# francescobrigante/Audio-Style-Transfer

Hardware: AMD Instinct MI355X
Metric: audio-seconds/sec/node (train step, 4s@22.05kHz pairs) (higher is better)
Workload: dtype bf16; 1 GPU; configs[1]: batch=8 4 s clips per GPU (S=2, x=(B,S,2,287,597)), full train2 step: STFT + CQT front-end from resident waveforms, encoders+decoder+discriminator, all losses, D and G phases, grad clip, Adam; global_batch=8, parallelism=dp1, hip_graph=True, dp_semantics=per-rank BN and batch-coupled losses

## Files before the change

audio-style-transfer_amd/ast_amd/ops.py:

```python
from __future__ import annotations

import ctypes
import functools
import math

import torch

from . import _lib, config
from ._lib import Gather, check, dcode, len_tensor, lib, ptr, stream


@functools.lru_cache(maxsize=None)
def const_tensor(values, dtype, device):
    return torch.tensor(values, dtype=dtype, device=device)


def pad8(c: int) -> int:
    return (c + 7) // 8 * 8


def _tap(dh, dw, wt):
    return (dh + 64) | ((dw + 64) << 8) | (wt << 16)


def _mk(N, Hs, Ws, Cs, Hm, Wm, sh, sw, oh, ow, Hd, Wd, Cd, dsh, dsw, doh, dow, taps, wtaps):
    g = Gather(N=N, Hs=Hs, Ws=Ws, Cs=Cs, Hm=Hm, Wm=Wm, sh=sh, sw=sw, oh=oh, ow=ow, Hd=Hd, Wd=Wd, Cd=Cd,
               dsh=dsh, dsw=dsw, doh=doh, dow=dow, ntaps=len(taps), wtaps=wtaps)
    for i, (dh, dw, wt) in enumerate(taps):
        g.tap[i] = _tap(dh, dw, wt)
    return g


@functools.lru_cache(maxsize=None)
def gather_direct(N, H, W, Cs, Cd, k, stride, pad):
    Ho = (H + 2 * pad - k) // stride + 1
    Wo = (W + 2 * pad - k) // stride + 1
    taps = tuple((kh, kw, kh * k + kw) for kh in range(k) for kw in range(k))
    return _mk(N, H, W, Cs, Ho, Wo, stride, stride, -pad, -pad, Ho, Wo, Cd, 1, 1, 0, 0, taps, k * k), (Ho, Wo)


@functools.lru_cache(maxsize=None)
def gathers_transposed(N, Hs, Ws, Cs, Hd, Wd, Cd, k, stride, pad):
    out = []
    for ph in range(stride):
        th = [((ph + pad - kh) // stride, kh) for kh in range(k) if (ph + pad - kh) % stride == 0]
        Hm = (Hd - ph + stride - 1) // stride
        for pw in range(stride):
            tw = [((pw + pad - kw) // stride, kw) for kw in range(k) if (pw + pad - kw) % stride == 0]
            Wm = (Wd - pw + stride - 1) // stride
            if Hm <= 0 or Wm <= 0:
                continue
            taps = tuple((dh, dw, kh * k + kw) for dh, kh in th for dw, kw in tw)
            out.append(_mk(N, Hs, Ws, Cs, Hm, Wm, 1, 1, 0, 0, Hd, Wd, Cd, stride, stride, ph, pw, taps, k * k))
    return tuple(out)


PROFILE = None


def _gemm_cost(g, esize, wgrad=False):
    M = g.N * g.Hm * g.Wm
    K = g.ntaps * g.Cs
    flops = 2.0 * M * g.Cd * K
    if wgrad:
        nbytes = (M * g.Cd + g.N * g.Hs * g.Ws * g.Cs) * esize + g.Cd * K * 4
    else:
        src_pix = min(g.N * g.Hs * g.Ws, M * max(g.ntaps, 1))
        nbytes = (src_pix * g.Cs + M * g.Cd + g.Cd * K) * esize
    return flops, nbytes


def _igemm_plan(g, dt):
    out = (ctypes.c_int32 * 5)()
    check(lib().ast_igemm_plan(g, dt, ctypes.byref(out)), "ast_igemm_plan")
    return out


def _igemm_config(g, dt):
    out = _igemm_plan(g, dt)
    if out[2] < 0:
        return f"patch{-out[0]}r{'(rows,' + str(-out[3]) + 'frag)' if out[3] < 0 else ''},{out[1]}ch,slab{-out[2]}B"
    return f"{out[0]}x{out[1]},k{out[2] * 16}B" + (f",split{out[3]}" if out[3] > 1 else "") + (f",kg{out[4]}" if out[4] > 1 else "")


_ws_cache = {}


def _ws_need(g, dt):
    det = config.deterministic
    key = (id(g), dt, det)
    v = _ws_cache.get(key)
    if v is None:
        v = int(lib().ast_igemm_ws_floats_det(g, dt) if det else lib().ast_igemm_ws_floats(g, dt))
        check(min(v, 0), "ast_igemm_ws_floats")
        _ws_cache[key] = v
    return v


STAT_SLOTS = 64


def stat_slots(C):
    s = STAT_SLOTS
    while s > 8 and s * C > 4096:
        s //= 2
    return s


def _slot_flags(slots):
    return 0 if slots == 64 else ((slots.bit_length() - 1) << _lib.IGEMM_SLOTS_SHIFT)


class _StatArena:
    CAP = 1 << 24
    by_device = {}


def stat_table(n, device):
    device = torch.device(device)
    a = _StatArena.by_device.get(device)
    if a is None:
        a = _StatArena.by_device[device] = [torch.zeros(_StatArena.CAP, dtype=torch.float32, device=device), 0, 0]
    n64 = (int(n) + 63) // 64 * 64
    if a[1] + n64 > _StatArena.CAP:
        if torch.cuda.is_current_stream_capturing():
            raise RuntimeError("statistics arena exhausted inside a hipGraph capture: call ops.stat_arena_reset() at the start of the step")
        torch.cuda.synchronize(device)
        a[0].zero_()
        a[1] = 0
    t = a[0][a[1]:a[1] + int(n)]
    a[1] += n64
    a[2] = max(a[2], a[1])
    return t


def stat_arena_reset(device):
    a = _StatArena.by_device.get(torch.device(device))
    if a is None or a[2] == 0:
        return
    if config.fused_finalize or _SyncBN.active:
        a[0][:a[2]].zero_()
    a[1] = 0


def stats_fusable(g, dt):
    return _ws_need(g, dt) == 0 and not config.deterministic


class BNLink:
    __slots__ = ("x", "scale", "shift", "relu", "table", "filled", "slots")

    def __init__(self):
        self.x = self.scale = self.shift = self.table = None
        self.relu, self.filled, self.slots = True, False, STAT_SLOTS


def in_stats_fusable(g, dt):
    return _igemm_plan(g, dt)[2] != 0 and _ws_need(g, dt) == 0 and not config.deterministic


def _igemm(src, wgt, bias, dst, g, flags=0, stats=None, bn=None, per_image=False):
    if PROFILE is not None:
        e0, e1 = torch.cuda.Event(enable_timing=True), torch.cuda.Event(enable_timing=True)
        e0.record()
# ... 1355 lines not shown
```

audio-style-transfer_amd/csrc/igemm.hip:

```cpp
#include "gemm_common.h"

namespace {


__device__ __forceinline__ int swz(int row, int c) { return ((c + (((row >> 3) & 1) << 1)) & 3) << 4; }

template <typename T>
struct EpiCtx {
  T* dst; const float* bias; float* ws; const T* bn_x; const float* bn_scale; const float* bn_shift;
  int HWm; float rcp_hw, rcp_w; bool accumulate, relu, stats, bstats, bn_relu;
};

template <typename T, int TN, int MODE>
__device__ __forceinline__ void epi_store_m(const EpiCtx<T>& ec, const ast_gather_t& g, const f32x4 (&col)[TN], const size_t pix, const int co0,
                                            float (&st1)[TN][4], float (&st2)[TN][4]) {
  T* drow = ec.dst + pix * g.Cd;
#pragma unroll
  for (int i = 0; i < TN; ++i) {
    const int co = co0 + i * 16;
    if (co >= g.Cd) continue;
    float v[4];
#pragma unroll
    for (int r = 0; r < 4; ++r) v[r] = col[i][r];
    if (ec.bias) {
// ... 376 lines not shown
  const int nks = (nchunks + 3) >> 2;
  const int HWm = g.Hm * g.Wm;
  const __amdgpu_buffer_rsrc_t srcR = __builtin_amdgcn_make_buffer_rsrc((void*)src, 0, src_bytes, 0x00020000);
  const __amdgpu_buffer_rsrc_t wgtR = __builtin_amdgcn_make_buffer_rsrc((void*)wgt, 0, wgt_bytes, 0x00020000);

  int sdelta[NKS], tdh[NKS], tdw[NKS];
  unsigned woff[NKS];
#pragma unroll
  for (int ks = 0; ks < NKS; ++ks) {
    const int kc = ks * 4 + fq;
    const bool kval = kc < nchunks;
    const int t = kval ? (cpc_shift >= 0 ? (kc >> cpc_shift) : kc / cpc) : 0;
    const int c0b = (kc - t * cpc) * 16;
    int dh, dw, wt;
    decode_tap(taptab[t], dh, dw, wt);
    sdelta[ks] = (dh * g.Ws + dw) * g.Cs * ES + c0b;
    tdh[ks] = kval ? dh : (1 << 20);
    tdw[ks] = dw;
    woff[ks] = kval ? (unsigned)(wt * g.Cs * ES + c0b) : OOB;
  }
  frag wreg[TN][NKS];
#pragma unroll
  for (int i = 0; i < TN; ++i) {
    const int co = bn0 + i * 16 + fr;
    const unsigned rowoff = co < g.Cd ? (unsigned)(co * g.wtaps * g.Cs * ES) : OOB;
#pragma unroll
    for (int ks = 0; ks < NKS; ++ks)
      wreg[i][ks] = __builtin_bit_cast(frag, __builtin_amdgcn_raw_buffer_load_b128(wgtR, (rowoff != OOB && woff[ks] != OOB) ? rowoff + woff[ks] : OOB, 0, 0));
  }

  const bool accumulate = flags & AST_IGEMM_ACCUMULATE, relu = flags & AST_IGEMM_RELU, stats = !DET && (flags & AST_IGEMM_STATS), bstats = !DET && (flags & AST_IGEMM_BN_SUMS), bn_relu = !(flags & AST_IGEMM_BN_NO_RELU);
  EpiCtx<T> ec{dst, bias, ws, bn_x, bn_scale, bn_shift, HWm, rcp_hw, rcp_w, accumulate, relu, stats, bstats, bn_relu};
  float st1[TN][4], st2[TN][4];
#pragma unroll
  for (int i = 0; i < TN; ++i)
#pragma unroll
    for (int r = 0; r < 4; ++r) { st1[i][r] = 0.f; st2[i][r] = 0.f; }

  auto load_pix = [&](int j, u32x4 (&xr)[NKS], int& dpix) __attribute__((always_inline)) {
    const int m = bm0 + j * 16 + fr;
    const bool valid = j < jt && m < M;
    const int mm = valid ? m : 0;
    const int n = fdiv(mm, HWm, rcp_hw), rem = mm - n * HWm;
    const int hm = fdiv(rem, g.Wm, rcp_w), wq = rem - hm * g.Wm;
    const int hs0 = valid ? hm * g.sh + g.oh : -(1 << 20);
    const int ws0 = wq * g.sw + g.ow;
    const int roff = (((n * g.Hs + (valid ? hs0 : 0)) * g.Ws + ws0) * g.Cs) * ES;
    dpix = (n * g.Hd + hm * g.dsh + g.doh) * g.Wd + (wq * g.dsw + g.dow);
#pragma unroll
    for (int ks = 0; ks < NKS; ++ks) {
      const bool ok = (unsigned)(hs0 + tdh[ks]) < (unsigned)g.Hs && (unsigned)(ws0 + tdw[ks]) < (unsigned)g.Ws;
      xr[ks] = __builtin_amdgcn_raw_buffer_load_b128(srcR, ok ? (unsigned)(roff + sdelta[ks]) : OOB, 0, 0);
    }
  };
  auto compute = [&](int j, const u32x4 (&xr)[NKS], const int dpix) __attribute__((always_inline)) {
    f32x4 acc[TN];
#pragma unroll
    for (int i = 0; i < TN; ++i) acc[i] = f32x4{0.f, 0.f, 0.f, 0.f};
#pragma unroll
    for (int ks = 0; ks < NKS; ++ks) {
      if (ks < nks) {
        const frag xf = __builtin_bit_cast(frag, xr[ks]);
#pragma unroll
        for (int i = 0; i < TN; ++i) acc[i] = Mma<T>::run(wreg[i][ks], xf, acc[i]);
      }
    }
    const int m = bm0 + j * 16 + fr;
    if (m < M) epi_store<T, TN>(ec, g, acc, (size_t)dpix, bn0 + fq * 4, st1, st2);
  };

  u32x4 xa[NKS], xb[NKS];
  int pa, pb;
  load_pix(0, xa, pa);
  for (int j = 0; j < jt; j += 2) {
    load_pix(j + 1, xb, pb);
    compute(j, xa, pa);
    load_pix(j + 2, xa, pa);
    if (j + 1 < jt) compute(j + 1, xb, pb);
  }
  __shared__ float red[(TN + 1) / 2 * 256];
  if (stats || bstats) epi_flush<T, TN>(ec, g, st1, st2, tix & stat_slot_mask(flags), bn0, fr, fq, red);
}

template <typename T>
__global__ __launch_bounds__(256) void splitk_finish_kernel(float* __restrict__ ws, const float* __restrict__ bias,
                                                            T* __restrict__ dst, const ast_gather_t g, const int M, const int flags,
                                                            const int nslabs) {
  const int c4 = g.Cd >> 2;
  const int HWm = g.Hm * g.Wm;
  const size_t total = (size_t)M * c4;
  for (size_t i = (size_t)blockIdx.x * 256 + threadIdx.x; i < total; i += (size_t)gridDim.x * 256) {
    const int m = (int)(i / c4), co = (int)(i % c4) * 4;
    const int n = m / HWm, rem = m - n * HWm;
    const int hm = rem / g.Wm, wq = rem - hm * g.Wm;
    const size_t pix = (size_t)(n * g.Hd + hm * g.dsh + g.doh) * g.Wd + (wq * g.dsw + g.dow);
    f32x4* wp = reinterpret_cast<f32x4*>(ws + (size_t)m * g.Cd + co);
    f32x4 a = *wp;
    if (nslabs > 0) {
      for (int z = 1; z < nslabs; ++z) a += *reinterpret_cast<const f32x4*>(ws + ((size_t)z * M + m) * g.Cd + co);
    } else {
      *wp = f32x4{0.f, 0.f, 0.f, 0.f};
    }
    float v[4] = {a[0], a[1], a[2], a[3]};
    if (bias) for (int r = 0; r < 4; ++r) v[r] += bias[co + r];
    store4<T>(dst + pix * g.Cd + co, v, flags & AST_IGEMM_ACCUMULATE, flags & AST_IGEMM_RELU);
  }
}

constexpr int PC_MAXPL = 8;

#ifdef AST_STAMPS
__device__ unsigned long long ast_stamps[16384 * 8];
#define PC_STAMP(k) do { if (threadIdx.x == 0 && tix < 16384) ast_stamps[tix * 8 + (k)] = (k) >= 6 ? wall_clock64() : __builtin_readcyclecounter(); } while (0)
#else
#define PC_STAMP(k) do { } while (0)
#endif
struct PconvPlan { int TH, TWF, PH, PW, dhmin, dwmin, tiles_h, tiles_w, nct, lds, rows, tm, wall; unsigned m_nct, m_per_img, m_tiles_w, m_pw20, m_twf, m_twf20; unsigned long long tapq[3]; };
__host__ __device__ __forceinline__ unsigned pc_magic(int d) { return d <= 1 ? 0u : (unsigned)((0x100000000ull + (unsigned)d - 1) / (unsigned)d); }
__device__ __forceinline__ int pc_div(int n, int d, unsigned m) { return d == 1 ? n : (int)__umulhi((unsigned)n, m); }
__device__ __forceinline__ int pc_div20(int n, unsigned m20) { return (int)(__umul24((unsigned)n, m20) >> 20); }

template <int SLB> __device__ __forceinline__ int pc_h(int p) { return SLB == 128 ? (p & 7) : ((p >> 1) & 3); }

typedef __attribute__((ext_vector_type(2))) unsigned int u32x2;
__device__ __forceinline__ f32x4 pc_as_f32x4(u32x4 u) {
  return __builtin_bit_cast(f32x4, u);
}
template <typename T>
__device__ __forceinline__ f32x4 pc_load4(__amdgpu_buffer_rsrc_t r, unsigned voff, int imm) {
  if constexpr (sizeof(T) == 4) {
    return pc_as_f32x4(__builtin_amdgcn_raw_buffer_load_b128(r, voff + (unsigned)imm, 0, 0));
  } else {
    const u32x2 u = __builtin_amdgcn_raw_buffer_load_b64(r, voff + (unsigned)imm, 0, 0);
    const u32x4 w{u.x << 16, u.x & 0xffff0000u, u.y << 16, u.y & 0xffff0000u};
    return __builtin_bit_cast(f32x4, w);
  }
}
template <typename T>
__device__ __forceinline__ void pc_store4(__amdgpu_buffer_rsrc_t r, unsigned voff, int imm, f32x4 v) {
  if constexpr (sizeof(T) == 4) {
    __builtin_amdgcn_raw_buffer_store_b128(__builtin_bit_cast(u32x4, v), r, voff + (unsigned)imm, 0, 0);
  } else {
    const bf16x4 q{(bf16_t)v[0], (bf16_t)v[1], (bf16_t)v[2], (bf16_t)v[3]};
    __builtin_amdgcn_raw_buffer_store_b64(__builtin_bit_cast(u32x2, q), r, voff + (unsigned)imm, 0, 0);
  }
}

template <typename T, int SLB, int TM, int TN, bool WALL, bool DET>
__global__ __launch_bounds__(256, (WALL ? 2 : (TM * TN <= 8 ? 4 : 2))) void pconv_kernel(const T* __restrict__ src, const T* __restrict__ wgt, const float* __restrict__ bias,
                                                    T* __restrict__ dst, const ast_gather_t g, const PconvPlan pp, const int flags,
                                                    float* __restrict__ ws, const unsigned src_bytes, const unsigned wgt_bytes,
                                                    const T* __restrict__ bn_x, const float* __restrict__ bn_scale,
                                                    const float* __restrict__ bn_shift) {
  constexpr int ES = sizeof(T);
  constexpr int CPP = SLB / 16;
  constexpr int BN = TN * 16;
  constexpr int NWL = (BN * CPP + 255) / 256;
  constexpr int KS = SLB / 64;
  constexpr unsigned OOB = 0x80000000u;
  using frag = typename Mma<T>::frag;
  extern __shared__ __attribute__((aligned(16))) unsigned char pl[];
  const int patch_bytes = pp.PH * pp.PW * SLB;
  unsigned char* wbuf = pl + patch_bytes;

  const int tid = threadIdx.x, lane = tid & 63, wave = tid >> 6;
  const int fr = lane & 15, fq = lane >> 4;
// ... 332 lines not shown
  if (best < 0.6) return false;
  pp.dhmin = dhmin; pp.dwmin = dwmin;
  const long spatial = (long)g.N * pp.tiles_h * pp.tiles_w;
  if (tn == 4 && spatial * ((g.Cd + 63) / 64) < 200) tn = 2;
  {
    const int mode = env_int("AST_PCONV_WALL", -1), nslab = rowb / slb;
    const int patch = pp.PH * pp.PW * slb;
    pp.wall = 0;
    if (dtype == AST_BF16 && g.ntaps >= 3 && mode != 0) {
      if (mode == 1) pp.wall = patch + g.ntaps * tn * 16 * slb <= 150 * 1024;
      else if ((mode == 2 || nslab >= 4) && patch + g.ntaps * 32 * slb <= 80 * 1024) { pp.wall = 1; tn = 2; }
    }
    pp.lds = patch + (pp.wall ? g.ntaps : 2) * tn * 16 * slb;
  }
  pp.nct = (g.Cd + tn * 16 - 1) / (tn * 16);
  pp.tapq[0] = pp.tapq[1] = pp.tapq[2] = 0;
  for (int t = 0; t < g.ntaps; ++t) {
    const int dh = (g.tap[t] & 255) - 64, dw = ((g.tap[t] >> 8) & 255) - 64, wt = g.tap[t] >> 16;
    const int toff = (dh - dhmin) * pp.PW + (dw - dwmin);
    if (toff >= 4096 || wt >= 16) return false;
    pp.tapq[t >> 2] |= (unsigned long long)(toff | (wt << 12)) << ((t & 3) * 16);
  }
  pp.m_nct = pc_magic(pp.nct); pp.m_per_img = pc_magic(pp.tiles_h * pp.tiles_w); pp.m_tiles_w = pc_magic(pp.tiles_w);
  pp.m_twf = pc_magic(pp.TWF);
  pp.m_pw20 = (unsigned)(((1u << 20) + pp.PW - 1) / pp.PW); pp.m_twf20 = (unsigned)(((1u << 20) + g.Wm - 1) / g.Wm);
  if ((double)g.N * pp.tiles_h * pp.tiles_w * pp.nct * std::max(pp.nct, pp.tiles_h * pp.tiles_w) >= 4294967296.0) return false;
  if (pp.PW >= 512 || g.Wm >= 512 || g.Ws >= (1 << 12) || g.Hs >= (1 << 12) || g.Cs * ES >= (1 << 13)) return false;
  if (spatial * pp.nct < env_int("AST_PCONV_MIN_TILES", 192)) return false;
  return pp.lds <= (pp.wall ? 150 : 64) * 1024;
}

struct IgemmPlan { int bm, bn, kch, nsplit, kt_per_split, depth, kgroups; };

IgemmPlan plan_igemm(const ast_gather_t& g, int M, int dtype) {
  const int E = dtype == AST_BF16 ? 8 : 4;
  const int nchunks = g.ntaps * (g.Cs / E);
  IgemmPlan p;
  if (g.Cd > 64) { p.bm = 64; p.bn = (M >= 30000) ? 128 : 64; }
  else if (g.Cd > 32) { p.bm = 64; p.bn = 64; }
  else if (g.Cd > 16) { p.bn = 32; p.bm = M >= 4096 ? 128 : 64; }
  else { p.bn = 16; p.bm = M >= 4096 ? 128 : 64; }
  p.kch = (p.bn >= 64 && nchunks >= 16) ? 8 : 4;
  const int KT = (nchunks + p.kch - 1) / p.kch;
  const long blocks = (long)((M + p.bm - 1) / p.bm) * ((g.Cd + p.bn - 1) / p.bn);
  p.nsplit = 1;
  p.kgroups = 1;
  static const long kg_blocks = getenv("AST_IGEMM_KG_BLOCKS") ? atol(getenv("AST_IGEMM_KG_BLOCKS")) : 400;
  static const int kg_kch = env_int("AST_IGEMM_KG_KCH", 8);
  if (p.bm == 64 && p.bn == 64 && blocks < kg_blocks && KT >= 16) { p.kgroups = 4; p.kch = kg_kch == 4 ? 4 : 8; }
  else if (blocks < 200 && KT >= 16 && (long)M * g.Cd <= (1L << 20)) p.nsplit = blocks < 120 ? 4 : 2;
  p.depth = 2;
  if (const char* f = getenv("AST_IGEMM_FORCE")) {
    int a, b, c, d, e = 0;
    const int nf = sscanf(f, "%d,%d,%d,%d,%d", &a, &b, &c, &d, &e);
    if (nf >= 4) { p.bm = a; p.bn = b; p.kch = c; p.nsplit = std::max(1, d); p.depth = 2; p.kgroups = 1; }
    if (nf >= 5) p.kgroups = (e == 4 && a == 64 && b == 64) ? 4 : 1;
  }
  {
    const int KT2 = (nchunks + p.kch - 1) / p.kch;
    p.nsplit = std::max(1, std::min(p.nsplit, std::max(1, KT2)));
    p.kt_per_split = (KT2 + p.nsplit - 1) / p.nsplit;
    p.nsplit = KT2 > 0 ? (KT2 + p.kt_per_split - 1) / p.kt_per_split : 1;
  }
  if (p.kt_per_split < 1) p.kt_per_split = 1;
  return p;
}

bool direct_ok(const ast_gather_t& g, const IgemmPlan& p, int dtype) {
  static const bool enabled = env_flag("AST_IGEMM_DIRECT", true);
  const int E = dtype == AST_BF16 ? 8 : 4;
  const int nchunks = g.ntaps * (g.Cs / E);
  static const int max_cd = env_int("AST_IGEMM_DIRECT_CD", 16);
  static const int max_chunks = env_int("AST_IGEMM_DIRECT_CHUNKS", 12);
  if ((long)g.N * g.Hd * g.Wd >= (1L << 31)) return false;
  return enabled && g.Cd <= std::min(max_cd, 32) && nchunks <= std::min(max_chunks, 12) && p.nsplit == 1 && p.kgroups == 1 &&
         !getenv("AST_IGEMM_FORCE");
}
int direct_jt(int M) {
  static const int env = env_int("AST_IGEMM_DIRECT_JT", 0);
  if (env > 0) return std::min(env, 64);
  return std::max(1, std::min(8, M / (64 * 2048)));
}

enum ConvKernel { CONV_PATCH, CONV_DIRECT, CONV_GATHERED };
struct ConvPlan {
  ConvKernel kernel; int M;
  IgemmPlan ig;
  PconvPlan pp; int slb, tn, TM;
  int jt, dtn, nks;
  long ws_plain, ws_det;
  bool split() const { return ws_plain > 0; }
};

ConvPlan plan_conv(const ast_gather_t& g, int dtype) {
  ConvPlan c{};
  c.M = g.N * g.Hm * g.Wm;
  if (plan_pconv(g, dtype, c.pp, c.slb, c.tn)) {
    c.kernel = CONV_PATCH;
    c.TM = c.slb == 128 ? (c.pp.tm == 1 || c.pp.tm == 2 ? c.pp.tm : 3) : (c.pp.tm == 2 || c.pp.tm == 4 ? c.pp.tm : 3);
    return c;
  }
  c.ig = plan_igemm(g, c.M, dtype);
  c.kernel = direct_ok(g, c.ig, dtype) ? CONV_DIRECT : CONV_GATHERED;
  if (c.kernel == CONV_DIRECT) { c.jt = direct_jt(c.M); c.dtn = g.Cd <= 16 ? 1 : 2; c.nks = std::max(1, (g.ntaps * (g.Cs / (dtype == AST_BF16 ? 8 : 4)) + 3) / 4); }
  if (c.ig.nsplit > 1) { c.ws_plain = (long)c.M * g.Cd; c.ws_det = c.ig.nsplit * c.ws_plain; }
  return c;
}

int check_conv_args(const ConvPlan& c, const ast_gather_t& g, int flags, const float* ws, long ws_floats, const void* bn_x,
                    const float* bn_scale, const float* bn_shift) {
  constexpr int STORE_MODS = AST_IGEMM_ACCUMULATE | AST_IGEMM_RELU;
  const long slots = stat_slot_mask(flags) + 1L;
  if ((flags & AST_IGEMM_DET) && (flags & (AST_IGEMM_STATS | AST_IGEMM_BN_SUMS | AST_IGEMM_PER_IMAGE)))
    AST_FAIL("ast_igemm: the deterministic form (flags bit 12) has no fused statistics (flags 8 / 16 / 64)");
  if (c.split()) {
    if (flags & (AST_IGEMM_STATS | AST_IGEMM_BN_SUMS)) AST_FAIL("ast_igemm: fused statistics (flags 8 / 16) are not available for a split-K plan (ast_igemm_ws_floats > 0)");
    const long need = (flags & AST_IGEMM_DET) ? c.ws_det : c.ws_plain;
    if (!ws || ws_floats < need) AST_FAIL("ast_igemm: this plan splits K and needs a workspace of %ld floats (ast_igemm_ws_floats%s), got %ld", need, (flags & AST_IGEMM_DET) ? "_det" : "", ws ? ws_floats : 0L);
  }
  if ((flags & AST_IGEMM_BN_SUMS) && ((flags & (STORE_MODS | AST_IGEMM_STATS)) || !ws || ws_floats < slots * g.Cd * 3 || !bn_x || !bn_scale || !bn_shift))
    AST_FAIL("ast_igemm: fused BatchNorm-backward sums need plain stores, a zeroed [slots][Cd][3] table and the layer's x / scale / shift");
  if ((flags & AST_IGEMM_STATS) && ((flags & STORE_MODS) || !ws || ws_floats < ((flags & AST_IGEMM_PER_IMAGE) ? (long)g.N : slots) * g.Cd * 2))
    AST_FAIL("ast_igemm: fused channel statistics need plain stores and a zeroed [slots][Cd][2] (per image: [N][Cd][2]) table");
  if ((flags & AST_IGEMM_PER_IMAGE) && (!(flags & AST_IGEMM_STATS) || c.split() || c.kernel == CONV_DIRECT))
    AST_FAIL("ast_igemm: per-image statistics (flag 64) need flag 8 and the patch or gathered kernel without split-K (ast_igemm_plan: kch != 0, no split)");
  return 0;
}

struct ConvCall {
  const void* src; const void* wgt; const float* bias; void* dst; ast_gather_t g; int flags; float* ws;
  const void* bn_x; const float* bn_scale; const float* bn_shift; hipStream_t s;
  unsigned src_bytes(size_t es) const { return (unsigned)((size_t)g.N * g.Hs * g.Ws * g.Cs * es); }
  unsigned wgt_bytes(size_t es) const { return (unsigned)((size_t)g.Cd * g.wtaps * g.Cs * es); }
  int chunk_shift(int E) const { const int cpc = g.Cs / E; int sh = -1; if ((cpc & (cpc - 1)) == 0) { sh = 0; while ((1 << sh) < cpc) ++sh; } return sh; }
};

template <typename T, int SLB, int TM, int TN, bool WALL>
int launch_pconv(const ConvCall& a, const ConvPlan& c) {
  const ast_gather_t& g = a.g; const PconvPlan& pp = c.pp;
  static LdsAttrOnce attr;
  if (int rc = attr.set((WALL ? 150 : 64) * 1024, {(const void*)pconv_kernel<T, SLB, TM, TN, WALL, false>, (const void*)pconv_kernel<T, SLB, TM, TN, WALL, true>})) return rc;
  const int tiles = g.N * pp.tiles_h * pp.tiles_w * pp.nct;
  const int grid = (tiles + 7) / 8 * 8;
  const auto k = (a.flags & AST_IGEMM_DET) ? pconv_kernel<T, SLB, TM, TN, WALL, true> : pconv_kernel<T, SLB, TM, TN, WALL, false>;
  hipLaunchKernelGGL(k, dim3(grid), dim3(256), pp.lds, a.s, (const T*)a.src, (const T*)a.wgt, a.bias, (T*)a.dst,
                     g, pp, a.flags, a.ws, a.src_bytes(sizeof(T)), a.wgt_bytes(sizeof(T)), (const T*)a.bn_x, a.bn_scale, a.bn_shift);
  AST_CHECK_LAUNCH();
  return 0;
}

template <typename T, int TN, int NKS>
int launch_direct(const ConvCall& a, const ConvPlan& c) {
  const ast_gather_t& g = a.g;
  const int tiles = ((c.M + 64 * c.jt - 1) / (64 * c.jt)) * ((g.Cd + TN * 16 - 1) / (TN * 16));
  const auto k = (a.flags & AST_IGEMM_DET) ? igemm_direct_kernel<T, TN, NKS, true> : igemm_direct_kernel<T, TN, NKS, false>;
  hipLaunchKernelGGL(k, dim3((tiles + 7) / 8 * 8), dim3(256), 0, a.s, (const T*)a.src, (const T*)a.wgt, a.bias, (T*)a.dst,
                     g, c.M, a.flags, a.ws, a.chunk_shift(16 / sizeof(T)), a.src_bytes(sizeof(T)), a.wgt_bytes(sizeof(T)),
                     1.0f / (float)(g.Hm * g.Wm), 1.0f / (float)g.Wm, (const T*)a.bn_x, a.bn_scale, a.bn_shift, c.jt);
  AST_CHECK_LAUNCH();
  return 0;
}

template <typename T, int BM, int BN, int WM, int WN, int KCH, int D, int KG, bool UT>
int launch_igemm_ut(const ConvCall& a, const ConvPlan& c) {
  const ast_gather_t& g = a.g; const IgemmPlan& p = c.ig; const int M = c.M, flags = a.flags;
  constexpr int LDS = KG * 2 * (KCH / 4) * (BM + BN) * 64 + 64;
  static_assert(KG == 1 || (KG - 1) * (BM / 16) * (BN / 16) / 4 * 256 * 16 <= KG * 2 * (KCH / 4) * (BM + BN) * 64, "reduce buffer fits");
  static LdsAttrOnce attr;
  if (int rc = attr.set(LDS, {(const void*)igemm_kernel<T, BM, BN, WM, WN, KCH, D, KG, UT, false>, (const void*)igemm_kernel<T, BM, BN, WM, WN, KCH, D, KG, UT, true>})) return rc;
  const int mtiles = (flags & AST_IGEMM_PER_IMAGE) ? g.N * ((g.Hm * g.Wm + BM - 1) / BM) : (M + BM - 1) / BM;
  const int tiles = mtiles * ((g.Cd + BN - 1) / BN);
  dim3 grid((tiles + 7) / 8 * 8, 1, p.nsplit);
  if (p.nsplit > 1 && !(flags & (AST_IGEMM_WS_ZEROED | AST_IGEMM_DET))) AST_HIP(hipMemsetAsync(a.ws, 0, sizeof(float) * (size_t)M * g.Cd, a.s));
  const auto k = (flags & AST_IGEMM_DET) ? igemm_kernel<T, BM, BN, WM, WN, KCH, D, KG, UT, true> : igemm_kernel<T, BM, BN, WM, WN, KCH, D, KG, UT, false>;
  hipLaunchKernelGGL(k, grid, dim3(256 * KG), LDS, a.s, (const T*)a.src, (const T*)a.wgt, a.bias, (T*)a.dst,
                     g, M, flags, a.ws, p.kt_per_split, a.chunk_shift(16 / sizeof(T)), a.src_bytes(sizeof(T)), a.wgt_bytes(sizeof(T)),
                     1.0f / (float)(g.Hm * g.Wm), 1.0f / (float)g.Wm, (const T*)a.bn_x, a.bn_scale, a.bn_shift);
  if (p.nsplit > 1) {
    const size_t total = (size_t)M * (g.Cd >> 2);
    hipLaunchKernelGGL((splitk_finish_kernel<T>), dim3((unsigned)std::min<size_t>((total + 255) / 256, 2048)), dim3(256), 0, a.s, a.ws, a.bias,
                       (T*)a.dst, g, M, flags, (flags & AST_IGEMM_DET) ? p.nsplit : 0);
  }
  AST_CHECK_LAUNCH();
  return 0;
}

template <typename T, int BM, int BN, int WM, int WN, int KCH, int D, int KG>
int launch_igemm(const ConvCall& a, const ConvPlan& c) {
  return a.g.Cs / (16 / (int)sizeof(T)) % KCH == 0 ? launch_igemm_ut<T, BM, BN, WM, WN, KCH, D, KG, true>(a, c) : launch_igemm_ut<T, BM, BN, WM, WN, KCH, D, KG, false>(a, c);
}

template <typename T>
int dispatch_conv(const ConvCall& a, const ConvPlan& c) {
  struct Entry { int k[4]; int (*fn)(const ConvCall&, const ConvPlan&); };
  auto run = [&](const Entry* tab, size_t n, int k0, int k1, int k2, int k3, const char* what) -> int {
    for (size_t i = 0; i < n; ++i) if (tab[i].k[0] == k0 && tab[i].k[1] == k1 && tab[i].k[2] == k2 && tab[i].k[3] == k3) return tab[i].fn(a, c);
    AST_FAIL("ast_igemm: no %s instantiation for the plan (%d, %d, %d, %d)", what, k0, k1, k2, k3);
  };
  if (c.kernel == CONV_PATCH) {
#define AST_PC(S_, M_, N_) {{S_, M_, N_, 0}, launch_pconv<T, S_, M_, N_, false>}, {{S_, M_, N_, 1}, launch_pconv<T, S_, M_, N_, true>}
    static const Entry tab[] = {AST_PC(128, 1, 4), AST_PC(128, 1, 2), AST_PC(128, 2, 4), AST_PC(128, 2, 2), AST_PC(128, 3, 4), AST_PC(128, 3, 2),
                                AST_PC(64, 2, 4),  AST_PC(64, 2, 2),  AST_PC(64, 4, 4),  AST_PC(64, 4, 2),  AST_PC(64, 3, 4),  AST_PC(64, 3, 2)};
#undef AST_PC
    return run(tab, sizeof(tab) / sizeof(tab[0]), c.slb, c.TM, c.tn, c.pp.wall, "pconv_kernel (SLB, TM, TN, WALL)");
  }
  if (c.kernel == CONV_DIRECT) {
#define AST_DK(TN_, K_) {{TN_, K_, 0, 0}, launch_direct<T, TN_, K_>}
    static const Entry tab[] = {AST_DK(1, 1), AST_DK(1, 2), AST_DK(1, 3), AST_DK(2, 1), AST_DK(2, 2), AST_DK(2, 3)};
#undef AST_DK
    return run(tab, sizeof(tab) / sizeof(tab[0]), c.dtn, c.nks, 0, 0, "igemm_direct_kernel (TN, NKS)");
  }
#define AST_IG(BM_, BN_, WM_, WN_, K_, KG_) {{BM_, BN_, K_, KG_}, launch_igemm<T, BM_, BN_, WM_, WN_, K_, 2, KG_>}
  static const Entry tab[] = {AST_IG(128, 128, 2, 2, 8, 1), AST_IG(128, 128, 2, 2, 4, 1), AST_IG(128, 64, 2, 2, 8, 1), AST_IG(128, 64, 2, 2, 4, 1),
                              AST_IG(64, 64, 2, 2, 8, 4),   AST_IG(64, 64, 2, 2, 4, 4),   AST_IG(64, 64, 2, 2, 8, 1),  AST_IG(64, 64, 2, 2, 4, 1),
                              AST_IG(64, 128, 1, 4, 8, 1),  AST_IG(64, 128, 1, 4, 4, 1),  AST_IG(128, 32, 4, 1, 4, 1), AST_IG(128, 16, 4, 1, 4, 1),
                              AST_IG(256, 32, 4, 1, 4, 1),  AST_IG(64, 32, 4, 1, 4, 1),   AST_IG(256, 16, 4, 1, 4, 1), AST_IG(64, 16, 4, 1, 4, 1)};
#undef AST_IG
  return run(tab, sizeof(tab) / sizeof(tab[0]), c.ig.bm, c.ig.bn, c.ig.kch, c.ig.kgroups, "igemm_kernel (BM, BN, KCH, KG)");
}

bool query_plan(const ast_gather_t* gp, int dtype, bool out_ok, const char* who, ConvPlan& c) {
  if (!gp || !out_ok || check_gather(gp, who)) return false;
  c = plan_conv(*gp, dtype);
  return true;
}

}

extern "C" long ast_igemm_ws_floats(const ast_gather_t* gp, int dtype) { ConvPlan c; return query_plan(gp, dtype, true, "ast_igemm_ws_floats", c) ? c.ws_plain : -1; }
extern "C" long ast_igemm_ws_floats_det(const ast_gather_t* gp, int dtype) { ConvPlan c; return query_plan(gp, dtype, true, "ast_igemm_ws_floats_det", c) ? c.ws_det : -1; }

extern "C" int ast_igemm_plan(const ast_gather_t* gp, int dtype, int* out5) {
  ConvPlan c;
  if (!query_plan(gp, dtype, out5 != nullptr, "ast_igemm_plan", c)) return -1;
  const int gathered[5] = {c.ig.bm, c.ig.bn, c.ig.kch, c.ig.nsplit, c.ig.kgroups};
  const int patch[5] = {-c.pp.TH, c.tn * 16, -c.slb, c.pp.rows ? -(c.pp.tm * 4) : 1, 1};
  const int direct[5] = {64 * c.jt, c.dtn * 16, 0, c.ig.nsplit, c.ig.kgroups};
  memcpy(out5, c.kernel == CONV_PATCH ? patch : c.kernel == CONV_DIRECT ? direct : gathered, sizeof(gathered));
  return 0;
}

extern "C" int ast_pconv_variant(const ast_gather_t* gp, int dtype, int* out4) {
  ConvPlan c;
  if (!query_plan(gp, dtype, out4 != nullptr, "ast_pconv_variant", c)) return -1;
  if (c.kernel != CONV_PATCH) return 0;
  out4[0] = c.slb; out4[1] = c.TM; out4[2] = c.tn; out4[3] = c.pp.wall;
  return 1;
}

extern "C" int ast_igemm_bn(const void* src, const void* wgt, const float* bias, void* dst, const ast_gather_t* gp,
                            int dtype, int flags, float* ws, long ws_floats, const void* bn_x, const float* bn_scale,
                            const float* bn_shift, void* stream) {
  if (int rc = check_gather(gp, "ast_igemm")) return rc;
  if (!src || !wgt || !dst) AST_FAIL("ast_igemm: null pointer");
  const ConvCall a{src, wgt, bias, dst, *gp, flags, ws, bn_x, bn_scale, bn_shift, (hipStream_t)stream};
  const ConvPlan c = plan_conv(a.g, dtype);
  if (int rc = check_conv_args(c, a.g, flags, ws, ws_floats, bn_x, bn_scale, bn_shift)) return rc;
  AST_DISPATCH_T(dtype, { return dispatch_conv<T>(a, c); });
}

extern "C" int ast_igemm(const void* src, const void* wgt, const float* bias, void* dst, const ast_gather_t* gp,
                         int dtype, int flags, float* ws, long ws_floats, void* stream) {
  return ast_igemm_bn(src, wgt, bias, dst, gp, dtype, flags & ~(AST_IGEMM_BN_SUMS | AST_IGEMM_BN_NO_RELU), ws, ws_floats, nullptr, nullptr, nullptr, stream);
}
```

Baseline: 5329 audio-seconds/sec.

## Add dedicated pointwise (1x1) conv kernel with register-resident weights and prefetch

Adds a specialized kernel for single-tap (1x1/strided shortcut) convolutions with moderate channel counts and large M. Weights are held in registers, source pixels are streamed with incremental address arithmetic and a multi-stage prefetch, and the existing epilogue (stats, BN sums, per-image stats) is reused. The intent is to replace the generic gathered igemm, which carries LDS staging and tile overhead, on these memory-bound layers. It adds more kernel variants and planning heuristics, and the new path could be slower for some shapes.

```diff
diff --git a/audio-style-transfer_amd/ast_amd/ops.py b/audio-style-transfer_amd/ast_amd/ops.py
--- a/audio-style-transfer_amd/ast_amd/ops.py
+++ b/audio-style-transfer_amd/ast_amd/ops.py
@@ -80,6 +80,8 @@
     out = _igemm_plan(g, dt)
     if out[2] < 0:
         return f"patch{-out[0]}r{'(rows,' + str(-out[3]) + 'frag)' if out[3] < 0 else ''},{out[1]}ch,slab{-out[2]}B"
+    if out[4] < 0:
+        return f"pointwise{out[0]}x{out[1]},k{out[2] * 16}B"
     return f"{out[0]}x{out[1]},k{out[2] * 16}B" + (f",split{out[3]}" if out[3] > 1 else "") + (f",kg{out[4]}" if out[4] > 1 else "")
 
 
diff --git a/audio-style-transfer_amd/csrc/igemm.hip b/audio-style-transfer_amd/csrc/igemm.hip
--- a/audio-style-transfer_amd/csrc/igemm.hip
+++ b/audio-style-transfer_amd/csrc/igemm.hip
@@ -482,6 +482,117 @@
   if (stats || bstats) epi_flush<T, TN>(ec, g, st1, st2, tix & stat_slot_mask(flags), bn0, fr, fq, red);
 }
 
+struct PwPlan {
+  int jt, runs, rpi;
+  int qw, rw;
+  int s16, d16;
+  int swrap_w, dwrap_w, swrap_h, dwrap_h;
+  int src0, wt;
+};
+
+template <typename T, int TN, int NKS, int MODE>
+__global__ __launch_bounds__(256) void pointwise_kernel(const T* __restrict__ src, const T* __restrict__ wgt,
+                                                        const float* __restrict__ bias, T* __restrict__ dst,
+                                                        const ast_gather_t g, const int M, const int flags,
+                                                        float* __restrict__ ws, const PwPlan pw,
+                                                        const unsigned src_bytes, const unsigned wgt_bytes,
+                                                        const float rcp_hw, const float rcp_w,
+                                                        const T* __restrict__ bn_x, const float* __restrict__ bn_scale,
+                                                        const float* __restrict__ bn_shift) {
+  constexpr int E = 16 / sizeof(T), ES = sizeof(T);
+  constexpr int PF = NKS == 1 ? 4 : (NKS == 2 ? 3 : 2);
+  constexpr unsigned OOB = 0x80000000u;
+  using frag = typename Mma<T>::frag;
+  const int lane = threadIdx.x & 63, wave = threadIdx.x >> 6;
+  const int fr = lane & 15, fq = lane >> 4;
+  const int NT = (g.Cd + TN * 16 - 1) / (TN * 16);
+  const int chunk = gridDim.x >> 3;
+  const int tix = (blockIdx.x & 7) * chunk + (blockIdx.x >> 3);
+  if (tix >= pw.runs * NT) return;
+  const int run = tix / NT, bn0 = (tix - run * NT) * TN * 16;
+  const bool per_image = flags & AST_IGEMM_PER_IMAGE;
+  const int HWm = g.Hm * g.Wm, jt = pw.jt;
+  const int img = per_image ? run / pw.rpi : 0;
+  const int m0 = (per_image ? img * HWm + (run - img * pw.rpi) * 64 * jt : run * 64 * jt) + wave * 16 * jt;
+  const int m_end = per_image ? (img + 1) * HWm : M;
+  const int cpc = g.Cs / E;
+  const __amdgpu_buffer_rsrc_t srcR = __builtin_amdgcn_make_buffer_rsrc((void*)src, 0, src_bytes, 0x00020000);
+  const __amdgpu_buffer_rsrc_t wgtR = __builtin_amdgcn_make_buffer_rsrc((void*)wgt, 0, wgt_bytes, 0x00020000);
+
+  frag wreg[TN][NKS];
+#pragma unroll
+  for (int i = 0; i < TN; ++i) {
+    const int co = bn0 + i * 16 + fr;
+#pragma unroll
+    for (int ks = 0; ks < NKS; ++ks) {
+      const int kc = ks * 4 + fq;
+      const unsigned off = (co < g.Cd && kc < cpc) ? (unsigned)(((co * g.wtaps + pw.wt) * g.Cs) * ES + kc * 16) : OOB;
+      wreg[i][ks] = __builtin_bit_cast(frag, __builtin_amdgcn_raw_buffer_load_b128(wgtR, off, 0, 0));
+    }
+  }
+
+  const bool accumulate = flags & AST_IGEMM_ACCUMULATE, relu = flags & AST_IGEMM_RELU, bn_relu = !(flags & AST_IGEMM_BN_NO_RELU);
+  EpiCtx<T> ec{dst, bias, ws, bn_x, bn_scale, bn_shift, HWm, rcp_hw, rcp_w, accumulate, relu, MODE == 1, MODE == 2, bn_relu};
+  float st1[TN][4], st2[TN][4];
+#pragma unroll
+  for (int i = 0; i < TN; ++i)
+#pragma unroll
+    for (int r = 0; r < 4; ++r) { st1[i][r] = 0.f; st2[i][r] = 0.f; }
+
+  int m = m0 + fr, hm, wq, dpix;
+  unsigned soff;
+  {
+    const int n = fdiv(m, HWm, rcp_hw), rem = m - n * HWm;
+    hm = fdiv(rem, g.Wm, rcp_w); wq = rem - hm * g.Wm;
+    soff = (unsigned)pw.src0 + (((unsigned)n * g.Hs + hm * g.sh) * g.Ws + wq * g.sw) * (unsigned)(g.Cs * ES);
+    dpix = (n * g.Hd + hm * g.dsh + g.doh) * g.Wd + (wq * g.dsw + g.dow);
+  }
+  unsigned koff[NKS];
+#pragma unroll
+  for (int ks = 0; ks < NKS; ++ks) koff[ks] = ks * 4 + fq < cpc ? (unsigned)((ks * 4 + fq) * 16) : OOB;
+
+  auto load_tile = [&](int j, u32x4 (&xr)[NKS], int& dp) __attribute__((always_inline)) {
+    const bool ok = j < jt && m < m_end;
+    dp = ok ? dpix : -1;
+#pragma unroll
+    for (int ks = 0; ks < NKS; ++ks)
+      xr[ks] = __builtin_amdgcn_raw_buffer_load_b128(srcR, (ok && koff[ks] != OOB) ? soff + koff[ks] : OOB, 0, 0);
+    m += 16; hm += pw.qw; wq += pw.rw; soff += (unsigned)pw.s16; dpix += pw.d16;
+    if (wq >= g.Wm) { wq -= g.Wm; ++hm; soff += (unsigned)pw.swrap_w; dpix += pw.dwrap_w; }
+    if (hm >= g.Hm) { hm -= g.Hm; soff += (unsigned)pw.swrap_h; dpix += pw.dwrap_h; }
+  };
+  auto compute = [&](const u32x4 (&xr)[NKS], const int dp) __attribute__((always_inline)) {
+    f32x4 acc[TN];
+#pragma unroll
+    for (int i = 0; i < TN; ++i) acc[i] = f32x4{0.f, 0.f, 0.f, 0.f};
+#pragma unroll
+    for (int ks = 0; ks < NKS; ++ks) {
+      const frag xf = __builtin_bit_cast(frag, xr[ks]);
+#pragma unroll
+      for (int i = 0; i < TN; ++i) acc[i] = Mma<T>::run(wreg[i][ks], xf, acc[i]);
+    }
+    if (dp >= 0) epi_store_m<T, TN, MODE>(ec, g, acc, (size_t)dp, bn0 + fq * 4, st1, st2);
+  };
+
+  u32x4 xr[PF][NKS];
+  int dp[PF];
+#pragma unroll
+  for (int st = 0; st < PF; ++st) load_tile(st, xr[st], dp[st]);
+  for (int j = 0; j < jt; j += PF) {
+#pragma unroll
+    for (int st = 0; st < PF; ++st) {
+      if (j + st < jt) {
+        compute(xr[st], dp[st]);
+        load_tile(j + st + PF, xr[st], dp[st]);
+      }
+    }
+  }
+  if constexpr (MODE != 0) {
+    __shared__ float red[(TN + 1) / 2 * 256];
+    epi_flush<T, TN>(ec, g, st1, st2, per_image ? ~img : (tix & stat_slot_mask(flags)), bn0, fr, fq, red);
+  }
+}
+
 template <typename T>
 __global__ __launch_bounds__(256) void splitk_finish_kernel(float* __restrict__ ws, const float* __restrict__ bias,
                                                             T* __restrict__ dst, const ast_gather_t g, const int M, const int flags,
@@ -980,7 +1091,22 @@
   return std::max(1, std::min(8, M / (64 * 2048)));
 }
 
-enum ConvKernel { CONV_PATCH, CONV_DIRECT, CONV_GATHERED };
+bool pointwise_ok(const ast_gather_t& g, const IgemmPlan& p, int M, int dtype) {
+  if (!env_flag("AST_POINTWISE", true) || getenv("AST_IGEMM_FORCE") || g.ntaps != 1) return false;
+  const int cpc = g.Cs / (dtype == AST_BF16 ? 8 : 4);
+  if (g.Cd <= 16 || g.Cd > 128 || g.Cs > 128 || cpc > 32 || p.nsplit != 1 || p.kgroups != 1) return false;
+  if (M < env_int("AST_POINTWISE_MIN_M", 131072) || g.Hm * g.Wm < 16) return false;
+  if ((long)g.N * g.Hd * g.Wd >= (1L << 31) || g.sh < 1 || g.sw < 1) return false;
+  const long h0 = g.oh + (g.tap[0] & 255) - 64, w0 = g.ow + ((g.tap[0] >> 8) & 255) - 64;
+  return h0 >= 0 && w0 >= 0 && (long)(g.Hm - 1) * g.sh + h0 < g.Hs && (long)(g.Wm - 1) * g.sw + w0 < g.Ws;
+}
+int pointwise_jt(int M) {
+  const int env = env_int("AST_POINTWISE_JT", 0);
+  if (env > 0) return std::min(env, 64);
+  return std::max(1, std::min(16, (M + 16 * 4096 - 1) / (16 * 4096)));
+}
+
+enum ConvKernel { CONV_PATCH, CONV_DIRECT, CONV_GATHERED, CONV_POINTWISE };
 struct ConvPlan {
   ConvKernel kernel; int M;
   IgemmPlan ig;
@@ -1001,6 +1127,13 @@
   c.ig = plan_igemm(g, c.M, dtype);
   c.kernel = direct_ok(g, c.ig, dtype) ? CONV_DIRECT : CONV_GATHERED;
   if (c.kernel == CONV_DIRECT) { c.jt = direct_jt(c.M); c.dtn = g.Cd <= 16 ? 1 : 2; c.nks = std::max(1, (g.ntaps * (g.Cs / (dtype == AST_BF16 ? 8 : 4)) + 3) / 4); }
+  else if (pointwise_ok(g, c.ig, c.M, dtype)) {
+    c.kernel = CONV_POINTWISE;
+    const int nks = (g.Cs / (dtype == AST_BF16 ? 8 : 4) + 3) / 4;
+    c.nks = nks <= 2 ? nks : (nks <= 4 ? 4 : 8);
+    c.dtn = (g.Cd <= 32 || c.nks == 8) ? 2 : 4;
+    c.jt = pointwise_jt(c.M);
+  }
   if (c.ig.nsplit > 1) { c.ws_plain = (long)c.M * g.Cd; c.ws_det = c.ig.nsplit * c.ws_plain; }
   return c;
 }
@@ -1021,7 +1154,7 @@
   if ((flags & AST_IGEMM_STATS) && ((flags & STORE_MODS) || !ws || ws_floats < ((flags & AST_IGEMM_PER_IMAGE) ? (long)g.N : slots) * g.Cd * 2))
     AST_FAIL("ast_igemm: fused channel statistics need plain stores and a zeroed [slots][Cd][2] (per image: [N][Cd][2]) table");
   if ((flags & AST_IGEMM_PER_IMAGE) && (!(flags & AST_IGEMM_STATS) || c.split() || c.kernel == CONV_DIRECT))
-    AST_FAIL("ast_igemm: per-image statistics (flag 64) need flag 8 and the patch or gathered kernel without split-K (ast_igemm_plan: kch != 0, no split)");
+    AST_FAIL("ast_igemm: per-image statistics (flag 64) need flag 8 and the patch, gathered or pointwise kernel without split-K (ast_igemm_plan: kch != 0, no split)");
   return 0;
 }
 
@@ -1055,6 +1188,36 @@
   hipLaunchKernelGGL(k, dim3((tiles + 7) / 8 * 8), dim3(256), 0, a.s, (const T*)a.src, (const T*)a.wgt, a.bias, (T*)a.dst,
                      g, c.M, a.flags, a.ws, a.chunk_shift(16 / sizeof(T)), a.src_bytes(sizeof(T)), a.wgt_bytes(sizeof(T)),
                      1.0f / (float)(g.Hm * g.Wm), 1.0f / (float)g.Wm, (const T*)a.bn_x, a.bn_scale, a.bn_shift, c.jt);
+  AST_CHECK_LAUNCH();
+  return 0;
+}
+
+template <typename T, int TN, int NKS>
+int launch_pointwise(const ConvCall& a, const ConvPlan& c) {
+  const ast_gather_t& g = a.g;
+  constexpr int ES = sizeof(T);
+  const int HWm = g.Hm * g.Wm, ppr = 64 * c.jt;
+  const bool per_image = a.flags & AST_IGEMM_PER_IMAGE;
+  PwPlan pw{};
+  pw.jt = c.jt;
+  pw.rpi = (HWm + ppr - 1) / ppr;
+  pw.runs = per_image ? g.N * pw.rpi : (c.M + ppr - 1) / ppr;
+  pw.qw = 16 / g.Wm; pw.rw = 16 % g.Wm;
+  const int spix = g.Cs * ES;
+  pw.s16 = (pw.qw * g.sh * g.Ws + pw.rw * g.sw) * spix;
+  pw.d16 = pw.qw * g.dsh * g.Wd + pw.rw * g.dsw;
+  pw.swrap_w = (g.sh * g.Ws - g.Wm * g.sw) * spix;
+  pw.dwrap_w = g.dsh * g.Wd - g.Wm * g.dsw;
+  pw.swrap_h = (g.Hs - g.Hm * g.sh) * g.Ws * spix;
+  pw.dwrap_h = (g.Hd - g.Hm * g.dsh) * g.Wd;
+  pw.src0 = ((g.oh + (g.tap[0] & 255) - 64) * g.Ws + g.ow + ((g.tap[0] >> 8) & 255) - 64) * spix;
+  pw.wt = g.tap[0] >> 16;
+  const int tiles = pw.runs * ((g.Cd + TN * 16 - 1) / (TN * 16));
+  const bool det = a.flags & AST_IGEMM_DET;
+  const auto k = (!det && (a.flags & AST_IGEMM_STATS)) ? pointwise_kernel<T, TN, NKS, 1> : (!det && (a.flags & AST_IGEMM_BN_SUMS)) ? pointwise_kernel<T, TN, NKS, 2> : pointwise_kernel<T, TN, NKS, 0>;
+  hipLaunchKernelGGL(k, dim3((tiles + 7) / 8 * 8), dim3(256), 0, a.s, (const T*)a.src, (const T*)a.wgt, a.bias, (T*)a.dst,
+                     g, c.M, a.flags, a.ws, pw, a.src_bytes(sizeof(T)), a.wgt_bytes(sizeof(T)),
+                     1.0f / (float)HWm, 1.0f / (float)g.Wm, (const T*)a.bn_x, a.bn_scale, a.bn_shift);
   AST_CHECK_LAUNCH();
   return 0;
 }
@@ -1108,6 +1271,12 @@
 #undef AST_DK
     return run(tab, sizeof(tab) / sizeof(tab[0]), c.dtn, c.nks, 0, 0, "igemm_direct_kernel (TN, NKS)");
   }
+  if (c.kernel == CONV_POINTWISE) {
+#define AST_PW(TN_, K_) {{TN_, K_, 0, 0}, launch_pointwise<T, TN_, K_>}
+    static const Entry tab[] = {AST_PW(2, 1), AST_PW(4, 1), AST_PW(2, 2), AST_PW(4, 2), AST_PW(2, 4), AST_PW(4, 4), AST_PW(2, 8)};
+#undef AST_PW
+    return run(tab, sizeof(tab) / sizeof(tab[0]), c.dtn, c.nks, 0, 0, "pointwise_kernel (TN, NKS)");
+  }
 #define AST_IG(BM_, BN_, WM_, WN_, K_, KG_) {{BM_, BN_, K_, KG_}, launch_igemm<T, BM_, BN_, WM_, WN_, K_, 2, KG_>}
   static const Entry tab[] = {AST_IG(128, 128, 2, 2, 8, 1), AST_IG(128, 128, 2, 2, 4, 1), AST_IG(128, 64, 2, 2, 8, 1), AST_IG(128, 64, 2, 2, 4, 1),
                               AST_IG(64, 64, 2, 2, 8, 4),   AST_IG(64, 64, 2, 2, 4, 4),   AST_IG(64, 64, 2, 2, 8, 1),  AST_IG(64, 64, 2, 2, 4, 1),
@@ -1134,7 +1303,8 @@
   const int gathered[5] = {c.ig.bm, c.ig.bn, c.ig.kch, c.ig.nsplit, c.ig.kgroups};
   const int patch[5] = {-c.pp.TH, c.tn * 16, -c.slb, c.pp.rows ? -(c.pp.tm * 4) : 1, 1};
   const int direct[5] = {64 * c.jt, c.dtn * 16, 0, c.ig.nsplit, c.ig.kgroups};
-  memcpy(out5, c.kernel == CONV_PATCH ? patch : c.kernel == CONV_DIRECT ? direct : gathered, sizeof(gathered));
+  const int pointwise[5] = {64 * c.jt, c.dtn * 16, gp->Cs / (dtype == AST_BF16 ? 8 : 4), 1, -c.nks};
+  memcpy(out5, c.kernel == CONV_PATCH ? patch : c.kernel == CONV_DIRECT ? direct : c.kernel == CONV_POINTWISE ? pointwise : gathered, sizeof(gathered));
   return 0;
 }
 
diff --git a/profiles/pointwise/ab_step.py b/profiles/pointwise/ab_step.py
--- /dev/null
+++ b/profiles/pointwise/ab_step.py
@@ -0,0 +1,37 @@
+#!/usr/bin/env python3
+import json
+import os
+import statistics
+import subprocess
+import sys
+
+HERE = os.path.dirname(os.path.dirname(os.path.dirname(os.path.abspath(__file__))))
+PARENT, ROUNDS = os.path.abspath(sys.argv[1]), int(sys.argv[2])
+NEW = os.path.join(HERE, "audio-style-transfer_amd", "ast_amd", "libast_hip.so")
+
+
+def bench(lib):
+    cmd = ["timeout", "-k", "10", "240", sys.executable, os.path.join(HERE, "bench.py"), "--gpus", "1", "--steps", "20", "--warmup", "5"]
+    r = subprocess.run(cmd, env=dict(os.environ, AST_HIP_LIB=lib), capture_output=True, text=True)
+    if r.returncode != 0:
+        sys.exit(f"bench.py with {lib}: exit {r.returncode}\n{r.stdout[-2000:]}\n{r.stderr[-2000:]}")
+    return json.loads([l for l in r.stdout.splitlines() if l.startswith("{")][-1])
+
+
+def main():
+    head = subprocess.run(["git", "-C", HERE, "rev-parse", "--short", "HEAD"], capture_output=True, text=True).stdout.strip() or sys.argv[3]
+    print(f"# parent = git head {head}; new = the same + working tree")
+    ms = {"parent": [], "new": []}
+    for r in range(ROUNDS):
+        for side, lib in (("parent", PARENT), ("new", NEW)):
+            res = bench(lib)
+            ms[side].append(res["ms_per_step"])
+            print(f"round {r + 1} {side:6s} ms_per_step {res['ms_per_step']:.4f}  " + " ".join(f"{k}={v}" for k, v in res.items() if "loss" in k), flush=True)
+    p, n = ms["parent"], ms["new"]
+    print(f"parent median {statistics.median(p):.4f} ({min(p):.4f}..{max(p):.4f}), spread {max(p) - min(p):.4f}")
+    print(f"new    median {statistics.median(n):.4f} ({min(n):.4f}..{max(n):.4f}), spread {max(n) - min(n):.4f}")
+    print(f"difference of medians {statistics.median(p) - statistics.median(n):.4f} ms; new max {'<' if max(n) < min(p) else '>='} parent min")
+
+
+if __name__ == "__main__":
+    main()
diff --git a/profiles/pointwise/isolated.py b/profiles/pointwise/isolated.py
--- /dev/null
+++ b/profiles/pointwise/isolated.py
@@ -0,0 +1,82 @@
+#!/usr/bin/env python3
+import os
+import statistics
+import subprocess
+import sys
+
+import torch
+
+HERE = os.path.dirname(os.path.dirname(os.path.dirname(os.path.abspath(__file__))))
+sys.path[:0] = [HERE, os.path.join(HERE, "audio-style-transfer_amd")]
+from ast_amd import _lib, ops
+
+DT = torch.bfloat16
+ROWS = [("b0 shortcut fwd 688896x32x8", "conv", 16, 288, 598, 8, 32, 2, "per_image"),
+        ("b1 shortcut fwd 172800x64x32", "conv", 16, 144, 299, 32, 64, 2, "per_image"),
+        ("b1 shortcut dgrad 172800x32x64", "dgrad", 16, 144, 299, 32, 64, 2, "accumulate"),
+        ("b2 shortcut fwd 43200x128x64", "conv", 16, 72, 150, 64, 128, 2, "per_image"),
+        ("b2 shortcut dgrad 43200x64x128", "dgrad", 16, 72, 150, 64, 128, 2, "accumulate"),
+        ("1x1 148608x32x64", "conv", 16, 72, 129, 64, 32, 1, "plain"),
+        ("1x1 32768x32x64", "conv", 16, 32, 64, 64, 32, 1, "plain"),
+        ("1x1 37440x64x64", "conv", 16, 36, 65, 64, 64, 1, "plain")]
+
+
+def setup(kind, N, H, W, Cs, Cd, stride):
+    if kind == "conv":
+        g, (Ho, Wo) = ops.gather_direct(N, H, W, Cs, Cd, 1, stride, 0)
+        return g, (N, H, W, Cs), (N, Ho, Wo, Cd), (Cd, 1, Cs)
+    Ho, Wo = (H - 1) // stride + 1, (W - 1) // stride + 1
+    g = ops.gathers_transposed(N, Ho, Wo, Cd, H, W, Cs, 1, stride, 0)[0]
+    return g, (N, Ho, Wo, Cd), (N, H, W, Cs), (Cs, 1, Cd)
+
+
+def time_row(g, sshape, dshape, wshape, form, reps=5):
+    fl, nbytes = ops._gemm_cost(g, 2)
+    nset = max(2, int(512 * 2 ** 20 / nbytes) + 1)
+    srcs = [torch.randn(sshape, device="cuda").to(DT) for _ in range(nset)]
+    dsts = [torch.zeros(dshape, device="cuda", dtype=DT) for _ in range(nset)]
+    w = (0.1 * torch.randn(wshape, device="cuda")).to(DT)
+    tabs = [torch.zeros(g.N * g.Cd * 2, device="cuda") for _ in range(nset)]
+
+    def launch(i):
+        if form == "per_image":
+            ops._igemm(srcs[i], w, None, dsts[i], g, stats=tabs[i], per_image=True)
+        else:
+            ops._igemm(srcs[i], w, None, dsts[i], g, flags=_lib.IGEMM_ACCUMULATE if form == "accumulate" else 0)
+
+    for i in range(nset):
+        launch(i)
+    torch.cuda.synchronize()
+    out = []
+    for _ in range(reps):
+        e0, e1 = torch.cuda.Event(enable_timing=True), torch.cuda.Event(enable_timing=True)
+        e0.record()
+        for i in range(nset):
+            launch(i)
+        e1.record()
+        torch.cuda.synchronize()
+        out.append(e0.elapsed_time(e1) * 1e3 / nset)
+    us = statistics.median(out)
+    return us, nbytes / us / 1e3, nbytes
+
+
+def main():
+    head = subprocess.run(["git", "-C", HERE, "rev-parse", "--short", "HEAD"], capture_output=True, text=True).stdout.strip() or "(no git)"
+    print(f"# git head {head} + working tree; {torch.cuda.get_device_name(0)}; bf16; us per launch (median of 5 series), GB/s vs algorithmic bytes")
+    jts = [int(a) for a in sys.argv[1:]]
+    for role, kind, N, H, W, Cs, Cd, stride, form in ROWS:
+        g, ss, ds, wsh = setup(kind, N, H, W, Cs, Cd, stride)
+        line = f"{role:34s} {form:10s}"
+        for sw, jt in [("0", 0), ("1", 0)] + [("1", j) for j in jts]:
+            os.environ["AST_POINTWISE"] = sw
+            os.environ.pop("AST_POINTWISE_JT", None)
+            if jt:
+                os.environ["AST_POINTWISE_JT"] = str(jt)
+            cfg = ops._igemm_config(g, _lib.dcode(DT))
+            us, gbs, nbytes = time_row(g, ss, ds, wsh, form)
+            line += f" | {cfg + (f' jt{jt}' if jt else ''):26s} {us:6.1f} us {gbs:5.0f} GB/s"
+        print(line + f" | {nbytes / 1e6:5.1f} MB", flush=True)
+
+
+if __name__ == "__main__":
+    main()
diff --git a/profiles/pointwise/resource_usage.py b/profiles/pointwise/resource_usage.py
--- /dev/null
+++ b/profiles/pointwise/resource_usage.py
@@ -0,0 +1,17 @@
+#!/usr/bin/env python3
+import re
+import subprocess
+import sys
+
+text = open(sys.argv[1]).read()
+head = subprocess.run(["git", "rev-parse", "--short", "HEAD"], capture_output=True, text=True).stdout.strip()
+print(f"# git head {head} (+ working tree); pointwise_kernel<T, TN, NKS, MODE>: MODE 0 plain / deterministic, 1 statistics, 2 BatchNorm-backward sums")
+print(f"{'dtype':5s} {'TN':>2s} {'NKS':>3s} {'MODE':>4s} {'VGPR':>5s} {'AGPR':>5s} {'scratch':>7s} {'LDS B':>6s} {'waves/SIMD':>10s}")
+for block in re.split(r"(?=remark: [^\n]*Function Name: )", text):
+    m = re.search(r"Function Name: \S*pointwise_kernelI(DF16b|f)Li(\d+)ELi(\d+)ELi(\d+)E", block)
+    if not m:
+        continue
+    f = lambda key: re.search(key + r": (\d+)", block).group(1)
+    scratch, lds, occ = f(r"ScratchSize \[bytes/lane\]"), f(r"LDS Size \[bytes/block\]"), f(r"Occupancy \[waves/SIMD\]")
+    print(f"{'bf16' if m.group(1) == 'DF16b' else 'f32':5s} {m.group(2):>2s} {m.group(3):>3s} {m.group(4):>4s} {f('VGPRs'):>5s} {f('AGPRs'):>5s} "
+          f"{scratch:>7s} {lds:>6s} {occ:>10s}")
```

New measurement: 5346 audio-seconds/sec (median of 6 runs). About the same (+0.3%).
